# mdnunez/bayesflow_nddms

Measured on AMD Instinct MI355X. Metric: simulated DDM trials/sec at n_trials=300 dt=0.001 (basic_ddm_dc, max_steps=4000), higher is better.
Workload: dtype f32

## Files before the change

bayesflow_nddms_amd/csrc/nddm_sim.h:

```cpp
#pragma once
#include <hip/hip_runtime.h>
#include <math.h>
#include <stdint.h>

#include "../../include/nddm.h"
#include "nddm_rng.h"

namespace nddm {

constexpr int WAVE = 64;
constexpr int MAX_REJECT = 64;

typedef __attribute__((address_space(3))) uint16_t lds_u16;
typedef __attribute__((address_space(3))) uint32_t lds_u32;
typedef uint32_t u32v4 __attribute__((ext_vector_type(4)));
typedef uint32_t u32v2 __attribute__((ext_vector_type(2)));
typedef __attribute__((address_space(3))) u32v4 lds_u32v4;
typedef __attribute__((address_space(3))) u32v2 lds_u32v2;

template <int MODEL> struct ModelTraits;
template <> struct ModelTraits<NDDM_BASIC_DDM_DC>      { static constexpr int P = 5; static constexpr bool HAS_Z = false; static constexpr int TAU = 3; };
template <> struct ModelTraits<NDDM_SINGLE_TRIAL>      { static constexpr int P = 8; static constexpr bool HAS_Z = true;  static constexpr int TAU = 3; };
template <> struct ModelTraits<NDDM_SINGLE_TRIAL_ALT>  { static constexpr int P = 8; static constexpr bool HAS_Z = true;  static constexpr int TAU = 3; };
template <> struct ModelTraits<NDDM_ALPHA_NOT_SCALED>  { static constexpr int P = 6; static constexpr bool HAS_Z = false; static constexpr int TAU = 3; };
template <> struct ModelTraits<NDDM_EXPLICIT_BOUNDARY> { static constexpr int P = 4; static constexpr bool HAS_Z = true;  static constexpr int TAU = 2; };

struct SimArgs {
    const float *params;
    const float *bounds;
    float *out_trials;
    float *out_summary;
    float *out_ext;
    uint16_t *out_codes;
    long long B;
    int n_trials;
    int n_total;
    int tiles_per_set;
    unsigned long long *partials;
    const uint32_t *recs;
    int max_k;
    float dt;
    float sqrt_dt;
    float tscale;
    uint32_t k0, k1;
    int sets_per_chunk;
    int n_chunks;
    unsigned int *chunk_counter;
    int ring;
    int open_ahead;
    float ext_sigma;
    int ext_mode;
    unsigned long long *dbg;
    int dbg_waves, dbg_chunks;
    int res16;
    int refill_thresh;
    uint32_t ring_magic;
    double dt64, sqrt_dt64;
};

typedef const __attribute__((address_space(4))) SimArgs *ArgsPtr;
__device__ __forceinline__ ArgsPtr fresh_args(ArgsPtr p)
{
    asm volatile("" : "+s"(p));
    return p;
}

template <bool FAST>
struct AuxStream {
    uint32_t trial, set_lo, c3, blk, kbase;
    u32x4 x;
    __device__ __forceinline__ AuxStream(uint32_t kbase_, uint32_t set_lo_, uint32_t set_hi28, uint32_t trial_)
        : trial(trial_), set_lo(set_lo_), c3(set_hi28 | 0x10000000u), blk(0xffffffffu), kbase(kbase_) {}
    __device__ __forceinline__ void block(uint32_t b)
    {
        if (b != blk) { x = philox4x32_10_lds(set_lo, trial, c3, b, kbase); blk = b; }
    }
    __device__ __forceinline__ void first_pair(float &z0, float &z1)
    {
        block(0u);
        float r, cs, sn;
        polar_pair<FAST>(x.x, x.y, r, cs, sn);
        r *= noise_unit<FAST>(1.0f);
        z0 = r * cs; z1 = r * sn;
    }
    __device__ __forceinline__ float normal(uint32_t a)
    {
        block(a >> 2);
        const bool second = (a & 2u) != 0u;
        float r, cs, sn;
        polar_pair<FAST>(second ? x.z : x.x, second ? x.w : x.y, r, cs, sn);
        r *= noise_unit<FAST>(1.0f);
        return r * ((a & 1u) ? sn : cs);
    }
};

__device__ __forceinline__ unsigned long long wave_sum(unsigned long long v)
{
#pragma unroll
    for (int off = 32; off > 0; off >>= 1) v += __shfl_xor(v, off, WAVE);
    return v;
}
__device__ __forceinline__ int wave_sum(int v)
{
#pragma unroll
    for (int off = 32; off > 0; off >>= 1) v += __shfl_xor(v, off, WAVE);
    return v;
}

__device__ __forceinline__ int fresh_lane(int lane)
{
    asm volatile("" : "+v"(lane));
    return lane;
}

__device__ __forceinline__ uint32_t lane_rank(unsigned long long mask)
{
    return __builtin_amdgcn_mbcnt_hi((uint32_t)(mask >> 32), __builtin_amdgcn_mbcnt_lo((uint32_t)mask, 0u));
}

__device__ __forceinline__ void finalize_summary(float *o, int n_up, int n_lo, int n_miss, unsigned long long sk,
                                                 unsigned long long sk2, unsigned long long sk_up,
                                                 unsigned long long sk2_up, long long sz, long long szz, int n_total,
                                                 float tscale, float tau)
{
    const double dtd = (double)tscale, taud = (double)tau;
    const double n_resp = (double)(n_up + n_lo);
    o[0] = (float)n_up; o[1] = (float)n_lo; o[2] = (float)n_miss;
    if (n_resp > 0) {
        const double mk = (double)sk / n_resp;
        const double vk = (double)sk2 / n_resp - mk * mk;
        o[3] = (float)(taud + dtd * mk);
        o[4] = (float)(dtd * dtd * vk);
    } else { o[3] = __builtin_nanf(""); o[4] = __builtin_nanf(""); }
    if (n_up > 0) {
        const double nu = (double)n_up;
        const double mk = (double)sk_up / nu;
        const double vk = (double)sk2_up / nu - mk * mk;
        o[5] = (float)(taud + dtd * mk);
        o[6] = (float)(dtd * dtd * vk);
    } else { o[5] = __builtin_nanf(""); o[6] = __builtin_nanf(""); }
    const double Nd = (double)n_total;
    const double mz = ((double)sz / 4294967296.0) / Nd;
    const double vz = ((double)szz / 16777216.0) / Nd - mz * mz;
    o[7] = (float)mz;
    o[8] = (float)vz;
    o[9] = (float)(((double)n_up + 0.5 * (double)n_miss) / Nd);
}

enum { REC = 12, R_A = 0, R_B = 4, R_SET = 8, R_TAU = 9, R_GLO = 10, R_GHI = 11 };

__device__ __forceinline__ void make_record(int model, bool fast, bool f64, const float *row, float dt, float sqrt_dt, int set,
                                            unsigned long long gset, uint32_t *r)
{
    float drift = 0.0f, a = 0.0f, beta = 0.0f, sig_c = 1.0f, tau;
    float b0 = 0.0f, b1 = 0.0f, b2 = 0.0f;
    switch (model) {
    case NDDM_BASIC_DDM_DC: drift = row[0]; a = row[1]; beta = row[2]; tau = row[3]; sig_c = row[4]; break;
    case NDDM_SINGLE_TRIAL: drift = row[0]; beta = row[2]; tau = row[3]; sig_c = row[5]; b0 = row[6]; b1 = row[7]; b2 = row[2]; break;
    case NDDM_SINGLE_TRIAL_ALT: tau = row[3]; b0 = row[5]; b1 = row[6]; b2 = row[7]; break;
    case NDDM_ALPHA_NOT_SCALED: a = row[1]; beta = row[2]; tau = row[3]; sig_c = row[5]; b0 = row[4]; break;
    default: drift = row[0]; beta = row[1]; tau = row[2]; sig_c = row[3]; break;
    }
    const float unit = sqrt_dt * sig_c;
    const float inv_s = 1.0f / (fast ? noise_unit<true>(unit) : noise_unit<false>(unit));
    const float hv = 0.5f * a;
    float a0 = (drift * dt) * inv_s, a1 = inv_s, a2 = hv * inv_s, a3 = (a * beta - hv) * inv_s;
    if (model == NDDM_SINGLE_TRIAL) { a2 = row[4]; a3 = row[1]; }
    else if (model == NDDM_SINGLE_TRIAL_ALT) { a0 = row[0]; a1 = row[1]; a2 = row[2]; a3 = row[4]; }
    else if (model == NDDM_ALPHA_NOT_SCALED) { a0 = row[0]; }
    else if (model == NDDM_EXPLICIT_BOUNDARY) { a2 = beta; a3 = 0.0f; }
    if (f64) {
        a0 = drift; a1 = sig_c;
        if (model == NDDM_BASIC_DDM_DC) { a2 = a; a3 = beta; }
    }
    r[0] = __float_as_uint(a0); r[1] = __float_as_uint(a1); r[2] = __float_as_uint(a2); r[3] = __float_as_uint(a3);
    r[4] = __float_as_uint(b0); r[5] = __float_as_uint(b1); r[6] = __float_as_uint(b2); r[7] = 0u;
    r[8] = (uint32_t)set; r[9] = __float_as_uint(tau);
    r[R_GLO] = (uint32_t)gset; r[R_GHI] = (uint32_t)(gset >> 32) & 0x0fffffffu;
}

enum { D_A = 0, D_B = 4,
       D_SIC = 8, D_TAU = 9, D_TBASE = 10, D_VSET = 11,
       D_CA = 12, D_CB = 13, D_HP1K = 14, D_X1 = 15,
       D_C3 = 16, D_SETLO = 17,
       D_ZSUM = 20,
       D_SPARE = 20 };
constexpr int DV = 24;
static_assert(D_SIC == R_SET && D_TAU == R_TAU, "the LDS record starts with the loaded record");
constexpr int LDS_HEADER_DWORDS = 32;
__host__ __device__ constexpr bool model_has_latent(int model)
{
    return model == NDDM_SINGLE_TRIAL || model == NDDM_SINGLE_TRIAL_ALT || model == NDDM_ALPHA_NOT_SCALED;
}
constexpr int LATENT_FIFO = 128;
__host__ __device__ constexpr int lds_header_bytes(int model)
{
    return LDS_HEADER_DWORDS * 4 + (model_has_latent(model) ? LATENT_FIFO * 4 : 0);
}
__host__ __device__ constexpr int slot_stride_bytes(int tile_trials, int bytes_per_result)
{
    return DV * 4 + ((tile_trials * bytes_per_result + 15) & ~15);
}

template <int MODEL, bool FAST>
__device__ __forceinline__ void trial_latent(const u32v4 dA, const u32v4 dB, uint32_t set_lo, uint32_t c3, uint32_t trial,
                                             uint32_t kbase, float &latent, float &z)
{
    static_assert(MODEL == NDDM_SINGLE_TRIAL || MODEL == NDDM_SINGLE_TRIAL_ALT, "models with a per-trial latent");
    const float sd = MODEL == NDDM_SINGLE_TRIAL ? __uint_as_float(dA.z) : __uint_as_float(dA.w);
    const float mean = MODEL == NDDM_SINGLE_TRIAL ? __uint_as_float(dA.w) : __uint_as_float(dB.x);
    const float sigma1 = MODEL == NDDM_SINGLE_TRIAL ? __uint_as_float(dB.x) : __uint_as_float(dB.y);
    const float gamma = MODEL == NDDM_SINGLE_TRIAL ? __uint_as_float(dB.y) : __uint_as_float(dB.z);
    AuxStream<FAST> aux(kbase, set_lo, c3, trial);
    float z0, z1;
    aux.first_pair(z0, z1);
    float v = __builtin_fmaf(sd, z1, mean);
    for (uint32_t ai = 2; !(v > 0.0f) && ai <= MAX_REJECT; ++ai) v = __builtin_fmaf(sd, aux.normal(ai), mean);
    if (!(v > 0.0f)) v = fabsf(v);
    latent = v;
    z = __builtin_fmaf(sigma1, z0, gamma * v);
}

template <bool FAST>
__device__ __forceinline__ float latent_normal_f64(const u32v4 dA, uint32_t set_lo, uint32_t c3, uint32_t trial, uint32_t kbase)
{
    const double sd = (double)__uint_as_float(dA.z), mean = (double)__uint_as_float(dA.w);
    AuxStream<FAST> aux(kbase, set_lo, c3, trial);
    float z0, z;
    aux.first_pair(z0, z);
    double v = mean + sd * (double)z;
    for (uint32_t ai = 2; !(v > 0.0) && ai <= MAX_REJECT; ++ai) { z = aux.normal(ai); v = mean + sd * (double)z; }
    return z;
}

__device__ __forceinline__ void z_fixed_point(float z, long long &fz, long long &fzz)
{
    z = fminf(fmaxf(z, -262144.0f), 262144.0f);
    const uint32_t b = __float_as_uint(z);
    const uint32_t e = (b >> 23) & 0xffu;
    const uint32_t m = (b & 0x007fffffu) | 0x00800000u;
    const uint32_t s1 = 147u - e, s2 = 291u - 2u * e;
    const unsigned long long mag = ((unsigned long long)m << 29) >> (s1 < 63u ? s1 : 63u);
    fz = (b >> 31) ? -(long long)mag : (long long)mag;
    fzz = (long long)((((unsigned long long)m * m) << 15) >> (s2 < 63u ? s2 : 63u));
}

template <int CTRL, int ROW_MASK>
__device__ __forceinline__ uint32_t dpp_add(uint32_t v)
{
    return v + (uint32_t)__builtin_amdgcn_update_dpp(0, (int)v, CTRL, ROW_MASK, 0xf, false);
}
__device__ __forceinline__ uint32_t wave_sum_dpp(uint32_t v)
{
    v = dpp_add<0x111, 0xf>(v);
    v = dpp_add<0x112, 0xf>(v);
    v = dpp_add<0x114, 0xf>(v);
    v = dpp_add<0x118, 0xf>(v);
    v = dpp_add<0x142, 0xa>(v);
    v = dpp_add<0x143, 0xc>(v);
    return v;
}

__host__ __device__ constexpr int partial_words(bool has_zsum) { return has_zsum ? 7 : 5; }

template <int MODEL, bool FAST, bool SMALL, bool CODES>
__device__ __forceinline__ void flush_set(ArgsPtr Ap, int lane, long long vset, uint32_t *d, const void *res, uint32_t kbase)
{
    using T = ModelTraits<MODEL>;
    constexpr bool ZSUM = MODEL == NDDM_SINGLE_TRIAL || MODEL == NDDM_SINGLE_TRIAL_ALT;
    const float tau = __uint_as_float(d[D_TAU]);
    [[maybe_unused]] u32v4 dA = {0u, 0u, 0u, 0u}, dB = {0u, 0u, 0u, 0u};
    [[maybe_unused]] uint32_t set_lo = 0u, c3 = 0u;
    [[maybe_unused]] long long acc_z = 0, acc_zz = 0;
    if constexpr (ZSUM) {
        dA = *reinterpret_cast<const u32v4 *>(d + D_A); dB = *reinterpret_cast<const u32v4 *>(d + D_B);
        c3 = d[D_C3]; set_lo = d[D_SETLO];
    }
    const int N = Ap->n_trials;
    const int TPS = Ap->tiles_per_set;
    const long long set_in_call = TPS == 1 ? vset : vset / TPS;
    const int t0 = TPS == 1 ? 0 : (int)(vset - set_in_call * TPS) * N;
    const int n_here = (Ap->n_total - t0) < N ? (Ap->n_total - t0) : N;
    uint32_t cnt2 = 0, sk32 = 0, sk2_32 = 0, sk_up32 = 0, sk2_up32 = 0;
    int n_up = 0, n_lo = 0, n_miss = 0;
    unsigned long long sk = 0, sk2 = 0, sk_up = 0, sk2_up = 0;
    float2 *out = Ap->out_trials ? reinterpret_cast<float2 *>(Ap->out_trials) + set_in_call * Ap->n_total + t0 : nullptr;
    static_assert(!CODES || (SMALL && (MODEL == NDDM_BASIC_DDM_DC || MODEL == NDDM_ALPHA_NOT_SCALED)), "wire-format kernels");
    constexpr bool HAS_CODES = CODES;
    [[maybe_unused]] uint16_t *codes = nullptr;
    if constexpr (HAS_CODES) { if (Ap->out_codes) codes = Ap->out_codes + set_in_call * Ap->n_total + t0; }
    for (uint32_t j = (uint32_t)lane; j < (uint32_t)n_here; j += WAVE) {
        uint32_t k, code;
        if (SMALL || Ap->res16) {
            const uint32_t v = static_cast<const uint16_t *>(res)[j];
            k = v & 0x3fffu; code = v >> 14;
            if constexpr (HAS_CODES) { if (codes) codes[j] = (uint16_t)v; }
        } else {
            const uint32_t v = static_cast<const uint32_t *>(res)[j];
            k = v & 0x3fffffffu; code = v >> 30;
        }
        const float ch = code == 1u ? 1.0f : (code == 2u ? -1.0f : 0.0f);
        const float rt = __builtin_fmaf((float)k, Ap->tscale, tau);
        float2 o;
        if constexpr (MODEL == NDDM_BASIC_DDM_DC) { o.x = rt; o.y = ch; }
        else if constexpr (MODEL == NDDM_ALPHA_NOT_SCALED) { o.x = ch * rt; o.y = 0.5f * (ch + 1.0f); }
        else {
            o.x = ch * rt;
            if constexpr (ZSUM) {
                float latent;
                trial_latent<MODEL, FAST>(dA, dB, set_lo, c3, (uint32_t)(t0 + j), kbase, latent, o.y);
                if (Ap->out_summary) { long long fz, fzz; z_fixed_point(o.y, fz, fzz); acc_z += fz; acc_zz += fzz; }
            } else {
                o.y = out ? Ap->bounds[set_in_call * Ap->n_total + t0 + j] : 0.0f;
            }
        }
        if constexpr (MODEL == NDDM_EXPLICIT_BOUNDARY) { if (code == 3u) o.x = __builtin_nanf(""); }
        if (out) out[j] = o;
        if (Ap->out_summary) {
            if constexpr (SMALL) {
                const uint32_t up01 = __builtin_amdgcn_ubfe(0x2u, code, 1u), resp01 = __builtin_amdgcn_ubfe(0x6u, code, 1u);
                const uint32_t kr = __umul24(k, resp01), ku = __umul24(k, up01);
                cnt2 += up01 | (resp01 << 10);
                sk32 += kr; sk_up32 += ku;
                sk2_32 = __umul24(kr, k) + sk2_32; sk2_up32 = __umul24(ku, k) + sk2_up32;
            } else {
                const unsigned long long kk = (unsigned long long)k * k;
                if (code == 1u) { n_up++; sk += k; sk2 += kk; sk_up += k; sk2_up += kk; }
                else if (code == 2u) { n_lo++; sk += k; sk2 += kk; }
                else n_miss++;
            }
        }
    }
    if (Ap->out_summary) {
        unsigned long long *q = reinterpret_cast<unsigned long long *>(Ap->partials) + vset * partial_words(ZSUM);
        [[maybe_unused]] unsigned long long *zsum = reinterpret_cast<unsigned long long *>(d + D_ZSUM);
        if constexpr (ZSUM) {
            atomicAdd(zsum, (unsigned long long)acc_z);
            atomicAdd(zsum + 1, (unsigned long long)acc_zz);
        }
        if constexpr (SMALL) {
            cnt2 = wave_sum_dpp(cnt2);
            sk32 = wave_sum_dpp(sk32); sk_up32 = wave_sum_dpp(sk_up32);
            const uint32_t a_hi = wave_sum_dpp(sk2_32 >> 16), a_lo = wave_sum_dpp(sk2_32 & 0xffffu);
            const uint32_t u_hi = wave_sum_dpp(sk2_up32 >> 16), u_lo = wave_sum_dpp(sk2_up32 & 0xffffu);
            if (fresh_lane(lane) == WAVE - 1) {
                const uint32_t n_up = cnt2 & 1023u, n_resp = cnt2 >> 10;
                q[0] = (unsigned long long)n_up | ((unsigned long long)(n_resp - n_up) << 21) |
                       ((unsigned long long)((uint32_t)n_here - n_resp) << 42);
                q[1] = sk32; q[2] = ((unsigned long long)a_hi << 16) + a_lo;
                q[3] = sk_up32; q[4] = ((unsigned long long)u_hi << 16) + u_lo;
                if constexpr (ZSUM) { q[5] = zsum[0]; q[6] = zsum[1]; }
            }
        } else {
            n_up = wave_sum(n_up); n_lo = wave_sum(n_lo); n_miss = wave_sum(n_miss);
            sk = wave_sum(sk); sk2 = wave_sum(sk2); sk_up = wave_sum(sk_up); sk2_up = wave_sum(sk2_up);
            if (fresh_lane(lane) == 0) {
                q[0] = (unsigned long long)n_up | ((unsigned long long)n_lo << 21) | ((unsigned long long)n_miss << 42);
                q[1] = sk; q[2] = sk2; q[3] = sk_up; q[4] = sk2_up;
                if constexpr (ZSUM) { q[5] = zsum[0]; q[6] = zsum[1]; }
            }
        }
    }
    if constexpr (MODEL == NDDM_ALPHA_NOT_SCALED) {
        if (Ap->out_ext && fresh_lane(lane) == 0 && t0 == 0) {
            AuxStream<FAST> aux(kbase, d[D_SETLO], d[D_C3], 0xffffffffu);
            const float loc = (Ap->ext_mode == 0) ? Ap->params[set_in_call * T::P + 1] : 1.0f;
            Ap->out_ext[set_in_call] = __builtin_fmaf(Ap->ext_sigma, aux.normal(0), loc);
        }
    }
}

__device__ __forceinline__ int ring_slot(int t, int ring, uint32_t magic)
{
    const uint32_t q = (uint32_t)(((unsigned long long)(uint32_t)t * magic) >> 32);
    int r = t - (int)(q * (uint32_t)ring);
    return r >= ring ? r - ring : r;
}

__device__ __forceinline__ bool in_range(float w, float h)
{
    return __builtin_fabsf(w) < h;
}


template <int MODEL, bool FAST, bool CAP4, bool BRIDGE, bool SMALL, bool PACKED, bool VKEYS, bool CODES = false, bool F64 = false>
__global__ __launch_bounds__(WAVE) void sim_kernel(const SimArgs A)
{
    static_assert(!F64 || ((MODEL == NDDM_BASIC_DDM_DC || MODEL == NDDM_SINGLE_TRIAL) && !BRIDGE && !PACKED && !VKEYS && !CODES),
                  "NDDM_STATE_F64 kernels");
    using T = ModelTraits<MODEL>;
    constexpr int P = T::P;
    extern __shared__ uint32_t lds_raw[];

    const ArgsPtr Ak = (ArgsPtr)__builtin_amdgcn_kernarg_segment_ptr();
    const int lane = threadIdx.x;
    const int N = A.n_trials;

    if (lane < 10) { lds_raw[2 * lane] = A.k0 + (uint32_t)lane * 0x9E3779B9u; lds_raw[2 * lane + 1] = A.k1 + (uint32_t)lane * 0xBB67AE85u; }
    if (lane == 0) { lds_raw[28] = A.k0 + 2u * PHILOX_W0; lds_raw[29] = A.k1 + 2u * PHILOX_W1; lds_raw[30] = A.k0 + 3u * PHILOX_W0; }
    uint32_t kbase;
    {
        const uint32_t off = (uint32_t)(size_t)lds_raw;
        asm volatile("v_mov_b32 %0, %1" : "=v"(kbase) : "s"(off));
    }
    const int rshift = SMALL ? 1 : (BRIDGE ? 2 : (A.res16 ? 1 : 2));
    constexpr bool LATENT = model_has_latent(MODEL);
    const int stride = DV * 4 + (((N << rshift) + 15) & ~15);
    char *const slots = reinterpret_cast<char *>(lds_raw) + lds_header_bytes(MODEL);
    auto slot_rec = [&](int slot) { return reinterpret_cast<uint32_t *>(slots + slot * stride); };
    auto pack_slots = [&](int t) {
        const ArgsPtr R = fresh_args(Ak);
        const int s0 = ring_slot(t, R->ring, R->ring_magic);
        const int o0 = s0 * stride, o01 = (s0 + 1 == R->ring ? 0 : s0 + 1) * stride - o0;
        return (o0 & 0xffff) | (o01 << 16);
    };
    constexpr uint32_t SLOTS_OFF = lds_header_bytes(MODEL);
    constexpr uint32_t FIFO_OFF = LDS_HEADER_DWORDS * 4;
    [[maybe_unused]] int fifo_pos = 0, fifo_avail = 0;

    float w = 0.0f, h = 0.0f, mu_dt = 0.0f;
    [[maybe_unused]] double xe = 0.0, ab = 0.0, cdt = 0.0, sdc = 0.0;
    int k = 0;
    [[maybe_unused]] float ta = 0.0f, tb = 0.0f;
    [[maybe_unused]] uint32_t jraw = 0;
    uint32_t res_addr = 0;
    [[maybe_unused]] int tile = 0;
    bool invalid = false;
    unsigned long long has_m = 0ull, act_m = 0ull;
    PathCtr pc = {0u, 0u, 0u, 0u, 0u};
    [[maybe_unused]] PathKeys pkeys;
    if constexpr (VKEYS) pkeys.init(A.k0, A.k1);

    int tile_open = 0;
    int flushed = 0;
    int next_tile = 0, next_trial = 0;
    int to_retire = N;
    int chunk_set = 0, chunk_left = 0;
    int slot_pack = pack_slots(0);
    int dirty = 1;
    unsigned long long dbg_cnt = 0;
    unsigned long long *dbg_stamp = reinterpret_cast<unsigned long long *>(lds_raw + 20);
    if (lane == 0) {
        dbg_stamp[3] = 0;
        lds_raw[31] = blockIdx.x;
        if (Ak->dbg) { dbg_stamp[0] = __builtin_amdgcn_s_memtime(); dbg_stamp[1] = __builtin_amdgcn_s_memrealtime(); }
    }

    uint32_t pre = 0u;

    auto open_tiles = [&]() {
        const ArgsPtr R = fresh_args(Ak);
        while (tile_open < flushed + R->ring && tile_open <= next_tile + R->open_ahead) {
            const bool have_pre = chunk_left > 0;
            if (chunk_left <= 0) {
                if (chunk_left < 0) break;
                unsigned int c = 0;
                if (fresh_lane(lane) == 0) c = atomicAdd(R->chunk_counter, 1u);
                c = __builtin_amdgcn_readfirstlane(c);
                if (c >= (unsigned int)R->n_chunks) {
                    chunk_left = -1;
                    if (fresh_lane(lane) == 0 && R->dbg) dbg_stamp[3] = __builtin_amdgcn_s_memrealtime();
                    break;
                }
                if (fresh_lane(lane) == 0 && R->dbg && c < (unsigned int)R->dbg_chunks)
                    R->dbg[8ll * R->dbg_waves + c] = __builtin_amdgcn_s_memrealtime();
                chunk_set = (int)c * R->sets_per_chunk;
                const long long left = R->B - (long long)chunk_set;
                chunk_left = (int)(left < R->sets_per_chunk ? left : R->sets_per_chunk);
            }
            const int slot = ring_slot(tile_open, R->ring, R->ring_magic);
            const int TPS = R->tiles_per_set;
            const int prow = TPS == 1 ? chunk_set : chunk_set / TPS;
            const int qt = chunk_set - prow * TPS;
            uint32_t rec = pre;
            if (!have_pre) rec = fresh_lane(lane) < REC ? R->recs[(long long)prow * REC + lane] : 0u;
            if (chunk_left > 1) {
                const int nrow = TPS == 1 ? chunk_set + 1 : (chunk_set + 1) / TPS;
                if (nrow != prow) pre = fresh_lane(lane) < REC ? R->recs[(long long)nrow * REC + lane] : 0u;
                else pre = rec;
            }
            const int sic = __builtin_amdgcn_readlane((int)rec, R_SET);
            const int vset = sic * TPS + qt;
            uint32_t *d = slot_rec(slot);
            if (lane < REC) d[lane] = rec;
            const uint32_t s_lo = (uint32_t)__builtin_amdgcn_readlane((int)rec, R_GLO);
            const uint32_t s_hi = (uint32_t)__builtin_amdgcn_readlane((int)rec, R_GHI);
            if (lane == 0) {
                d[D_VSET] = (uint32_t)vset;
                if constexpr (MODEL == NDDM_SINGLE_TRIAL || MODEL == NDDM_SINGLE_TRIAL_ALT) { d[D_ZSUM] = 0u; d[D_ZSUM + 1] = 0u; d[D_ZSUM + 2] = 0u; d[D_ZSUM + 3] = 0u; }
                PathSet ps;
                ps.init(s_lo, s_hi, R->k0, R->k1);
                d[D_CA] = ps.cA; d[D_CB] = ps.cB; d[D_HP1K] = ps.hP1k; d[D_X1] = ps.X1;
                d[D_SETLO] = s_lo;
                d[D_C3] = s_hi;
                d[D_TBASE] = (uint32_t)(qt * N);
            }
            chunk_set++; chunk_left--; tile_open++;
        }
    };

    while (true) {
        const unsigned long long fin_mask0 = has_m & ~act_m;
        if (__builtin_amdgcn_inverse_ballot_w64(fin_mask0)) {
            uint32_t code = invalid ? 3u : (w >= h ? 1u : (w <= -h ? 2u : 0u));
            if constexpr (F64) code = xe >= ab ? 1u : (xe <= 0.0 ? 2u : 0u);
            uint32_t tfix = (uint32_t)k;
            if constexpr (BRIDGE) {
                const bool started = fmaxf(ta, tb) > 0.0f;
                const bool stepped = started && k < A.max_k;
                code = (stepped || !started) ? (w >= 0.0f ? 1u : 2u) : 0u;
                const uint32_t jit = (k & 1) ? ((jraw >> 16) & 0xffu) : (jraw & 0xffu);
                tfix = (((uint32_t)k + (stepped ? 1u : 0u)) << 8) - (stepped ? jit : 0u);
            }
            if (SMALL || rshift == 1) *reinterpret_cast<lds_u16 *>(res_addr + (SLOTS_OFF + DV * 4)) = (uint16_t)(tfix | (code << 14));
            else *reinterpret_cast<lds_u32 *>(res_addr + (SLOTS_OFF + DV * 4)) = tfix | (code << 30);
        }
        has_m &= ~fin_mask0;
        to_retire -= (int)__popcll(fin_mask0);
        if (to_retire <= 0) {
            __syncthreads();
            while (flushed < tile_open) {
                if (next_tile <= flushed) break;
                const int fslot = ring_slot(flushed, fresh_args(Ak)->ring, fresh_args(Ak)->ring_magic);
                if constexpr (SMALL) {
                    const uint32_t fsb = (uint32_t)(fslot * stride) + kbase;
                    if (__builtin_amdgcn_ballot_w64(res_addr - fsb < (uint32_t)stride) & has_m) break;
                } else {
                    if (__builtin_amdgcn_ballot_w64(tile == flushed) & has_m) break;
                }
                uint32_t *const d = slot_rec(fslot);
                const int set_in_call = __builtin_amdgcn_readfirstlane((int)d[D_VSET]);
                flush_set<MODEL, FAST, SMALL, CODES>(fresh_args(Ak), lane, (long long)set_in_call, d, d + DV, kbase);
                flushed++;
                to_retire += N;
                dirty = 1;
            }
            __syncthreads();
        }
        if (dirty) {
            dirty = 0;
            if (tile_open <= next_tile + fresh_args(Ak)->open_ahead && tile_open < flushed + fresh_args(Ak)->ring && chunk_left >= 0) {
                open_tiles();
                __syncthreads();
            }
            if (flushed == tile_open && chunk_left < 0) break;
        }
        {
            const unsigned long long want_mask = ~has_m;
            int tr = next_trial + (int)lane_rank(want_mask);
            int tl = next_tile;
            while (tr >= N) { tr -= N; tl++; }
            const unsigned long long ok_mask = want_mask & __builtin_amdgcn_ballot_w64(tl < tile_open);
            const int off0 = slot_pack & 0xffff, off01 = slot_pack >> 16;
            const int tile0 = next_tile;
            if constexpr (LATENT) {
                const int n_ok = (int)__popcll(ok_mask);
                if (n_ok > fifo_avail) {
                    int btr = next_trial + fifo_avail + lane, btl = next_tile;
                    while (btr >= N) { btr -= N; btl++; }
                    const unsigned long long bmask = __builtin_amdgcn_ballot_w64(btl < tile_open);
                    if (__builtin_amdgcn_inverse_ballot_w64(bmask)) {
                        const uint32_t bsb = (uint32_t)(__mul24(btl - tile0, off01) + off0) + kbase;
                        const lds_u32v4 *const bq = reinterpret_cast<const lds_u32v4 *>(bsb + SLOTS_OFF);
                        const u32v4 dA = bq[D_A / 4];
                        [[maybe_unused]] const u32v4 dB = bq[D_B / 4];
                        const u32v4 dS = bq[D_SIC / 4];
                        const u32v2 sw = *reinterpret_cast<const lds_u32v2 *>(bsb + SLOTS_OFF + D_C3 * 4);
                        const uint32_t btrial = (uint32_t)btr + dS.z;
                        float v;
                        if constexpr (MODEL == NDDM_ALPHA_NOT_SCALED) {
                            AuxStream<FAST> aux(kbase, sw.y, sw.x, btrial);
                            v = (__builtin_fmaf(__uint_as_float(dB.x), aux.normal(0), __uint_as_float(dA.x)) * fresh_args(Ak)->dt) * __uint_as_float(dA.y);
                        } else if constexpr (F64) {
                            v = latent_normal_f64<FAST>(dA, sw.y, sw.x, btrial, kbase);
                        } else {
                            float z_unused;
                            trial_latent<MODEL, FAST>(dA, dB, sw.y, sw.x, btrial, kbase, v, z_unused);
                        }
                        *reinterpret_cast<__attribute__((address_space(3))) float *>(
                            kbase + FIFO_OFF + (((uint32_t)(fifo_pos + fifo_avail + lane) & (LATENT_FIFO - 1)) << 2)) = v;
                    }
                    fifo_avail += (int)__popcll(bmask);
                }
            }
            next_trial += (int)__popcll(ok_mask);
            if (next_trial >= N) {
                const int ring_bytes = fresh_args(Ak)->ring * stride;
                int o0 = slot_pack & 0xffff, o01 = slot_pack >> 16;
                while (next_trial >= N) {
                    next_trial -= N; next_tile++;
                    o0 += o01;
                    o01 = o0 + stride == ring_bytes ? -o0 : stride;
                }
                slot_pack = (o0 & 0xffff) | (o01 << 16);
                dirty = 1;
            }
            has_m |= ok_mask;
            if (__builtin_amdgcn_inverse_ballot_w64(ok_mask)) {
#ifdef NDDM_EXTRA_REFILL_VALU
                { uint32_t dummy = (uint32_t)lane;
#pragma unroll
                  for (int e = 0; e < NDDM_EXTRA_REFILL_VALU; ++e) asm volatile("v_xor_b32 %0, 0x55, %0" : "+v"(dummy)); }
#endif
                const ArgsPtr H = fresh_args(Ak);
                if constexpr (!SMALL) tile = tl;
                const uint32_t sb = (uint32_t)(__mul24(tl - tile0, off01) + off0) + kbase;
                res_addr = sb + ((uint32_t)tr << rshift);
                const lds_u32v4 *const rq = reinterpret_cast<const lds_u32v4 *>(sb + SLOTS_OFF);
                const lds_u32 *const rw = reinterpret_cast<const lds_u32 *>(sb + SLOTS_OFF);
                const u32v4 d0 = rq[D_A / 4];
                const u32v4 d1 = rq[D_CA / 4];
                const u32v4 d2 = rq[D_SIC / 4];
                const float a0 = __uint_as_float(d0.x), a1 = __uint_as_float(d0.y), a2 = __uint_as_float(d0.z),
                            a3 = __uint_as_float(d0.w);
                const uint32_t trial = (uint32_t)tr + d2.z;
                [[maybe_unused]] float latent = 0.0f;
                if constexpr (LATENT)
                    latent = *reinterpret_cast<const __attribute__((address_space(3))) float *>(
                        kbase + FIFO_OFF + (((uint32_t)fifo_pos + lane_rank(want_mask)) & (LATENT_FIFO - 1)) * 4u);
                invalid = false;
                if constexpr (F64) {
                    double beta64;
                    if constexpr (MODEL == NDDM_BASIC_DDM_DC) { ab = (double)a2; beta64 = (double)a3; }
                    else {
                        ab = (double)a3 + (double)a2 * (double)latent;
                        if (!(ab > 0.0)) ab = __builtin_fabs(ab);
                        beta64 = (double)__uint_as_float(rw[D_B + 2]);
                    }
                    xe = ab * beta64;
                    cdt = (double)a0 * H->dt64;
                    sdc = H->sqrt_dt64 * (double)a1;
                    if constexpr (FAST) sdc *= 1.1774100225154747;
                } else if constexpr (MODEL == NDDM_BASIC_DDM_DC) {
                    mu_dt = a0; h = a2; w = a3;
                } else if constexpr (MODEL == NDDM_SINGLE_TRIAL) {
                    const float a = latent;
                    const float hv = 0.5f * a;
                    mu_dt = a0;
                    h = hv * a1;
                    w = (a * __uint_as_float(rw[D_B + 2]) - hv) * a1;
                } else if constexpr (MODEL == NDDM_SINGLE_TRIAL_ALT) {
                    const float sig_c = latent;
                    const float inv_t = 1.0f / noise_unit<FAST>(H->sqrt_dt * sig_c);
                    const float hv = 0.5f * a1;
                    mu_dt = (a0 * H->dt) * inv_t;
                    h = hv * inv_t;
                    w = (a1 * a2 - hv) * inv_t;
                } else if constexpr (MODEL == NDDM_ALPHA_NOT_SCALED) {
                    mu_dt = latent;
                    h = a2; w = a3;
                } else if constexpr (MODEL == NDDM_EXPLICIT_BOUNDARY) {
                    const float a = trial < (uint32_t)H->n_total ? H->bounds[(long long)d2.x * H->n_total + trial] : 1.0f;
                    invalid = !(a >= 0.0f);
                    const float hv = 0.5f * a;
                    mu_dt = a0;
                    h = invalid ? 0.0f : hv * a1;
                    w = (a * a2 - hv) * a1;
                }
                const uint4 kq = *reinterpret_cast<const uint4 *>(lds_raw + 28);
                pc.init(d1.x, d1.y, d1.z, d1.w, trial, kq.x, kq.y, kq.z);
                k = 0;
                if constexpr (BRIDGE) { ta = h - __builtin_fabsf(w); tb = ta; jraw = 0u; }
            }
            if constexpr (LATENT) { const int n_ok = (int)__popcll(ok_mask); fifo_pos += n_ok; fifo_avail -= n_ok; }
            if constexpr (BRIDGE) act_m = __builtin_amdgcn_ballot_w64(ta > 0.0f) & __builtin_amdgcn_ballot_w64(k < A.max_k) & has_m;
            else if constexpr (F64) act_m = __builtin_amdgcn_ballot_w64(xe > 0.0) & __builtin_amdgcn_ballot_w64(xe < ab) & __builtin_amdgcn_ballot_w64(k < A.max_k) & has_m;
            else act_m = __builtin_amdgcn_ballot_w64(in_range(w, h)) & __builtin_amdgcn_ballot_w64(k < A.max_k) & has_m;
        }
        constexpr int MAX_BLOCKS = 16;
        const int it_limit = A.refill_thresh < WAVE ? MAX_BLOCKS - 1 : 0x7fffffff;
        const int occupied = (int)__popcll(has_m);
        const int leave_at = occupied < A.refill_thresh ? occupied : A.refill_thresh;
        int it = 0;
        for (;; ++it) {
            if constexpr (BRIDGE) {
                const uint32_t blk = (uint32_t)k;
                const u32x4 u4 = philox4x32_10_path(blk | 0x80000000u, pc, kbase);
                unsigned long long &live = act_m;
#pragma unroll
                for (int half = 0; half < 2; ++half) {
                    const u32x4 rb = philox4x32_10_path(blk + 4u * (uint32_t)half, pc, kbase);
                    float r0, r1, c0, c1, c2, c3;
                    polar_pair<FAST, true>(rb.x, rb.y, r0, c0, c1);
                    polar_pair<FAST, true>(rb.z, rb.w, r1, c2, c3);
                    const uint32_t ua = half ? u4.z : u4.x, ub = half ? u4.w : u4.y;
                    if constexpr (FAST && CAP4) {
                        float m, uf;
#define NDDM_BSTEP(R, T, D0, D1, CVT, KLIT) "v_fmac_f32 %[w], %[" R "], %[" T "]\n\tv_add_f32 %[w], %[mu], %[w]\n\tv_sub_f32 %[" D1 "], %[h], |%[w]|\n\t" \
    "v_mul_f32 %[m], %[" D0 "], %[" D1 "]\n\tv_fmaak_f32 %[m], -4.0, %[m], " KLIT "\n\tv_exp_f32 %[m], %[m]\n\t" CVT                        \
    "v_cmpx_ge_f32_e64 vcc, %[uf], %[m]\n\tv_add_u32 %[k], 1, %[k]\n\t"
#define NDDM_U32(W) "v_cvt_f32_u32 %[uf], %[" W "]\n\t"
#define NDDM_U16(W) "v_and_b32 %[uf], 0xffff, %[" W "]\n\tv_cvt_f32_u32 %[uf], %[uf]\n\t"
                        asm volatile("s_mov_b64 exec, %[lm]\n\t"
                                     "v_mov_b32 %[jr], %[ua]\n\t"
                                     NDDM_BSTEP("r0", "c0", "ta", "tb", NDDM_U32("ua"), "0x42000001")
                                     NDDM_BSTEP("r0", "c1", "tb", "ta", NDDM_U16("ua"), "0x41800000")
                                     "v_mov_b32 %[jr], %[ub]\n\t"
                                     NDDM_BSTEP("r1", "c2", "ta", "tb", NDDM_U32("ub"), "0x42000001")
                                     NDDM_BSTEP("r1", "c3", "tb", "ta", NDDM_U16("ub"), "0x41800000")
                                     "s_nop 1\n\ts_mov_b64 %[lm], exec\n\ts_mov_b64 exec, -1"
                                     : [w] "+v"(w), [k] "+v"(k), [ta] "+v"(ta), [tb] "+v"(tb), [jr] "+v"(jraw), [lm] "+s"(live), [m] "=&v"(m),
                                       [uf] "=&v"(uf)
                                     : [mu] "v"(mu_dt), [h] "v"(h), [r0] "v"(r0), [r1] "v"(r1), [c0] "v"(c0), [c1] "v"(c1),
                                       [c2] "v"(c2), [c3] "v"(c3), [ua] "v"(ua), [ub] "v"(ub)
                                     : "vcc");
#undef NDDM_BSTEP
#undef NDDM_U32
#undef NDDM_U16
                    } else {
                        bool active = __builtin_amdgcn_inverse_ballot_w64(live);
                        const float rr4[4] = {r0, r0, r1, r1}, tt4[4] = {c0, c1, c2, c3};
#pragma unroll
                        for (int j = 0; j < 4; ++j) {
                            if (active) {
                                asm volatile("" ::: "memory");
                                const uint32_t word = j < 2 ? ua : ub;
                                const float w1 = __builtin_fmaf(rr4[j], tt4[j], w) + mu_dt;
                                const float t1 = h - __builtin_fabsf(w1);
                                const float m = ((j & 1) ? tb : ta) * t1;
                                if (j & 1) ta = t1; else tb = t1;
                                if ((j & 1) == 0) jraw = word;
                                const float uf = (j & 1) ? (float)(word & 0xffffu) : (float)word;
                                bool cross;
                                if constexpr (FAST) {
                                    const float kk = (j & 1) ? 16.0f : __uint_as_float(0x42000001u);
                                    cross = !(uf >= __builtin_amdgcn_exp2f(__builtin_fmaf(-4.0f, m, kk)));
                                } else {
                                    const float u = uf * ((j & 1) ? 1.52587890625e-05f : 2.3283064365386963e-10f);
                                    cross = !(t1 > 0.0f) || u < exact_expf_neg(-2.0f * m);
                                }
                                w = w1;
                                if (cross) active = false;
                                else {
                                    k++;
                                    if constexpr (!CAP4) active = k < A.max_k;
                                }
                            }
                        }
                        live = __builtin_amdgcn_ballot_w64(active);
                    }
                }
                act_m &= __builtin_amdgcn_ballot_w64(k < A.max_k);
                if ((int)__popcll(has_m & ~act_m) >= leave_at) break;
                if (it >= it_limit) break;
                continue;
            }
            [[maybe_unused]] bool active = (CAP4 && !PACKED && !F64) ? false : __builtin_amdgcn_inverse_ballot_w64(act_m);
            constexpr int NS = PACKED ? 8 : 4;
            const uint32_t blk = (uint32_t)k;
            u32x4 rb;
            if constexpr (VKEYS) rb = philox4x32_10_path(blk, pc, pkeys);
            else rb = philox4x32_10_path(blk, pc, kbase);
            float rr[NS], tt[NS];
            if constexpr (PACKED) {
                polar_pair_packed<FAST>(rb.x, rr[0], tt[0], tt[1]);
                polar_pair_packed<FAST>(rb.y, rr[2], tt[2], tt[3]);
                polar_pair_packed<FAST>(rb.z, rr[4], tt[4], tt[5]);
                polar_pair_packed<FAST>(rb.w, rr[6], tt[6], tt[7]);
                rr[1] = rr[0]; rr[3] = rr[2]; rr[5] = rr[4]; rr[7] = rr[6];
            } else {
                polar_pair<FAST, true>(rb.x, rb.y, rr[0], tt[0], tt[1]);
                polar_pair<FAST, true>(rb.z, rb.w, rr[2], tt[2], tt[3]);
                rr[1] = rr[0]; rr[3] = rr[2];
            }
            if constexpr (F64) {
#pragma unroll
                for (int j = 0; j < NS; ++j) {
                    if (active) {
                        asm volatile("" ::: "memory");
                        const double zn = (double)rr[j] * (double)tt[j];
                        xe = xe + (cdt + sdc * zn);
                        k++;
                        if (j < NS - 1) {
                            if constexpr (CAP4) active = (xe > 0.0) && (xe < ab);
                            else active = (xe > 0.0) && (xe < ab) && (k < A.max_k);
                        }
                    }
                }
                act_m = __builtin_amdgcn_ballot_w64(xe > 0.0) & __builtin_amdgcn_ballot_w64(xe < ab) & __builtin_amdgcn_ballot_w64(k < A.max_k) & has_m;
                if ((int)__popcll(has_m & ~act_m) >= leave_at) break;
                if (it >= it_limit) break;
                continue;
            }
            if constexpr (CAP4 && !PACKED) {
                unsigned long long still;
#define NDDM_STEP(R, T) "v_fmac_f32 %[w], %[" R "], %[" T "]\n\tv_add_f32 %[w], %[mu], %[w]\n\tv_add_u32 %[k], 1, %[k]\n\tv_cmpx_lt_f32_e64 vcc, |%[w]|, %[h]\n\t"
                asm volatile("s_mov_b64 exec, %[am]\n\t"
                             NDDM_STEP("r0", "t0") NDDM_STEP("r0", "t1") NDDM_STEP("r1", "t2") NDDM_STEP("r1", "t3")
                             "s_nop 1\n\ts_mov_b64 %[st], exec\n\ts_mov_b64 exec, -1"
                             : [w] "+v"(w), [k] "+v"(k), [st] "=s"(still)
                             : [am] "s"(act_m), [mu] "v"(mu_dt), [h] "v"(h), [r0] "v"(rr[0]), [r1] "v"(rr[2]),
                               [t0] "v"(tt[0]), [t1] "v"(tt[1]), [t2] "v"(tt[2]), [t3] "v"(tt[3])
                             : "vcc");
#undef NDDM_STEP
                act_m = still & __builtin_amdgcn_ballot_w64(k < A.max_k);
                if ((int)__popcll(has_m & ~act_m) >= leave_at) break;
                if (it >= it_limit) break;
                continue;
            }
#pragma unroll
            for (int j = 0; j < NS; ++j) {
                if (active) {
                    asm volatile("" ::: "memory");
                    w = __builtin_fmaf(rr[j], tt[j], w) + mu_dt;
                    k++;
                    if (j < NS - 1) {
                        if constexpr (CAP4) active = in_range(w, h);
                        else active = in_range(w, h) && (k < A.max_k);
                    }
                }
            }
            act_m = __builtin_amdgcn_ballot_w64(in_range(w, h)) & __builtin_amdgcn_ballot_w64(k < A.max_k) & has_m;
            if ((int)__popcll(has_m & ~act_m) >= leave_at) break;
            if (it >= it_limit) break;
        }
        dbg_cnt += (1ull << 32) | (unsigned long long)(uint32_t)(it + 1);
    }
    if (lane == 0) {
        unsigned int *const q = fresh_args(Ak)->chunk_counter;
        const unsigned int left = atomicAdd(q + 1, 1u);
        if (left == gridDim.x - 1u) { atomicExch(q, 0u); atomicExch(q + 1, 0u); }
    }
    unsigned long long *const dbg = fresh_args(Ak)->dbg;
    if (dbg && lane == 0) {
        const unsigned long long t_end = __builtin_amdgcn_s_memrealtime(), c_end = __builtin_amdgcn_s_memtime();
        const uint32_t wg = lds_raw[31];
        if (wg < (uint32_t)fresh_args(Ak)->dbg_waves) {
            unsigned long long *const r = dbg + 8ull * wg;
            r[0] = dbg_cnt & 0xffffffffull; r[1] = dbg_cnt >> 32;
            r[2] = c_end - dbg_stamp[0]; r[3] = t_end - dbg_stamp[1];
            r[4] = dbg_stamp[1]; r[5] = dbg_stamp[3]; r[6] = t_end; r[7] = 1ull;
        }
    }
}

}
```

Before: 9.308 billion.

## Halve step counter increments and skip max_k ballot unless near cap

The inline-asm 4-step walk now increments k by 2 every two steps and tracks which lanes exited after an odd step with s_xor masks, correcting only those lanes afterwards. The per-iteration k<max_k ballot is replaced by a check that runs only when some lane in the wave is within 4*MAX_BLOCKS steps of max_k, decided once at refill time. This cuts per-step VALU and per-iteration SALU/ballot overhead in the hot loop, at the cost of more intricate exec-mask bookkeeping and a possible correctness risk in step-count accounting.

```diff
diff --git a/bayesflow_nddms_amd/csrc/nddm_sim.h b/bayesflow_nddms_amd/csrc/nddm_sim.h
--- a/bayesflow_nddms_amd/csrc/nddm_sim.h
+++ b/bayesflow_nddms_amd/csrc/nddm_sim.h
@@ -427,6 +427,8 @@
     [[maybe_unused]] int tile = 0;
     bool invalid = false;
     unsigned long long has_m = 0ull, act_m = 0ull;
+    constexpr int MAX_BLOCKS = 16;
+    [[maybe_unused]] int cap_k = -1;
     PathCtr pc = {0u, 0u, 0u, 0u, 0u};
     [[maybe_unused]] PathKeys pkeys;
     if constexpr (VKEYS) pkeys.init(A.k0, A.k1);
@@ -665,9 +667,14 @@
             if constexpr (LATENT) { const int n_ok = (int)__popcll(ok_mask); fifo_pos += n_ok; fifo_avail -= n_ok; }
             if constexpr (BRIDGE) act_m = __builtin_amdgcn_ballot_w64(ta > 0.0f) & __builtin_amdgcn_ballot_w64(k < A.max_k) & has_m;
             else if constexpr (F64) act_m = __builtin_amdgcn_ballot_w64(xe > 0.0) & __builtin_amdgcn_ballot_w64(xe < ab) & __builtin_amdgcn_ballot_w64(k < A.max_k) & has_m;
+            else if constexpr (CAP4 && !PACKED) {
+                const int max_k = fresh_args(Ak)->max_k;
+                act_m = max_k > 0 ? __builtin_amdgcn_ballot_w64(in_range(w, h)) & has_m : 0ull;
+                const int near_from = A.refill_thresh < WAVE ? max_k - 4 * MAX_BLOCKS : (int)0x80000000;
+                cap_k = (__builtin_amdgcn_ballot_w64(k >= near_from) & has_m) ? max_k : -1;
+            }
             else act_m = __builtin_amdgcn_ballot_w64(in_range(w, h)) & __builtin_amdgcn_ballot_w64(k < A.max_k) & has_m;
         }
-        constexpr int MAX_BLOCKS = 16;
         const int it_limit = A.refill_thresh < WAVE ? MAX_BLOCKS - 1 : 0x7fffffff;
         const int occupied = (int)__popcll(has_m);
         const int leave_at = occupied < A.refill_thresh ? occupied : A.refill_thresh;
@@ -783,17 +790,30 @@
                 continue;
             }
             if constexpr (CAP4 && !PACKED) {
-                unsigned long long still;
-#define NDDM_STEP(R, T) "v_fmac_f32 %[w], %[" R "], %[" T "]\n\tv_add_f32 %[w], %[mu], %[w]\n\tv_add_u32 %[k], 1, %[k]\n\tv_cmpx_lt_f32_e64 vcc, |%[w]|, %[h]\n\t"
+#define NDDM_STEP(R, T, K2) "v_fmac_f32 %[w], %[" R "], %[" T "]\n\tv_add_f32 %[w], %[mu], %[w]\n\t" K2 "v_cmpx_lt_f32_e64 vcc, |%[w]|, %[h]\n\t"
+#define NDDM_K2 "v_add_u32 %[k], 2, %[k]\n\t"
                 asm volatile("s_mov_b64 exec, %[am]\n\t"
-                             NDDM_STEP("r0", "t0") NDDM_STEP("r0", "t1") NDDM_STEP("r1", "t2") NDDM_STEP("r1", "t3")
-                             "s_nop 1\n\ts_mov_b64 %[st], exec\n\ts_mov_b64 exec, -1"
-                             : [w] "+v"(w), [k] "+v"(k), [st] "=s"(still)
-                             : [am] "s"(act_m), [mu] "v"(mu_dt), [h] "v"(h), [r0] "v"(rr[0]), [r1] "v"(rr[2]),
+                             NDDM_STEP("r0", "t0", NDDM_K2) "s_xor_b64 %[am], %[am], vcc\n\t"
+                             NDDM_STEP("r0", "t1", "")      "s_xor_b64 %[am], %[am], vcc\n\t"
+                             NDDM_STEP("r1", "t2", NDDM_K2) "s_xor_b64 %[am], %[am], vcc\n\t"
+                             NDDM_STEP("r1", "t3", "")      "s_andn2_b64 %[am], %[am], vcc\n\t"
+                             "s_cbranch_scc0 1f\n\t"
+                             "s_mov_b64 exec, %[am]\n\t"
+                             "v_subrev_u32 %[k], 1, %[k]\n"
+                             "1:\n\t"
+                             "s_mov_b64 %[am], vcc\n\t"
+                             "s_mov_b64 exec, -1\n\t"
+                             "s_cmp_lt_i32 %[ck], 0\n\t"
+                             "s_cbranch_scc1 2f\n\t"
+                             "v_cmp_gt_i32 vcc, %[ck], %[k]\n\t"
+                             "s_and_b64 %[am], %[am], vcc\n"
+                             "2:"
+                             : [w] "+v"(w), [k] "+v"(k), [am] "+s"(act_m)
+                             : [ck] "s"(cap_k), [mu] "v"(mu_dt), [h] "v"(h), [r0] "v"(rr[0]), [r1] "v"(rr[2]),
                                [t0] "v"(tt[0]), [t1] "v"(tt[1]), [t2] "v"(tt[2]), [t3] "v"(tt[3])
-                             : "vcc");
+                             : "vcc", "scc");
 #undef NDDM_STEP
-                act_m = still & __builtin_amdgcn_ballot_w64(k < A.max_k);
+#undef NDDM_K2
                 if ((int)__popcll(has_m & ~act_m) >= leave_at) break;
                 if (it >= it_limit) break;
                 continue;
```

Result: faster. 9.592 billion, median of 6 (+3.0%).
